# kdexd/virtex

Measured on NVIDIA H100. Metric: image-caption pairs/sec bicaptioning R50-L1-H1024, higher is better.
Workload: dtype bf16

## Files before the change

virtex_b200/csrc/gemm_tc.cu:

```cuda
#include <stdlib.h>
#include "ptx.cuh"
#include "vtx_common.cuh"
#include "../../include/virtex_b200.h"

#define KP_TAPS_W p.taps_w
#define KP_PAD p.pad
#define KP_NTAPS p.ntaps

namespace vtx {

constexpr int kBM = 128;
constexpr int kBK = 64;
constexpr int kMaxStages = 8;
constexpr int kABytes = kBM * kBK * 2;
constexpr int kSmemTotal = 232448;
constexpr int kCtrlBytes = 1024;
constexpr int kThreads = 384;
constexpr int kEpiThreads = 256;

struct FastDiv {
  uint32_t mul, shr;
};
__device__ __forceinline__ int fdiv(int x, const FastDiv& f) {
  return f.mul == 0u ? x : (int)(__umulhi((uint32_t)x, f.mul) >> f.shr);
// ... 18 lines not shown
  int bn;
  int a_mn, b_mn;
  int m_tiles, n_tiles, k_splits;
  int kb_total, kb_per_split;
  int mode;
  int cH, cW, cN, cpb;
  int lbw, lbh, lbn;
  int tiles_w, tiles_h;
  int out_f32, atomic, act;
  int stages, stage_bytes;
  int cbytes, nbuf;
  int res_tma;
  float alpha;
  void* D;
  long long ldd;
  const float* bias;
  int bias_pairs;
  const __nv_bfloat16* residual;
  long long ldr;
  const uint8_t* res_mask;
  float* stats;
  int taps_w, pad, ntaps;
  int cstride;
  FastDiv d_mn, d_nt, d_mt, d_tw, d_twh, d_cpb, d_taps;
  unsigned int* sched;
  unsigned int sched_base;
  int sched_chunk;
  int nt_major;
  const __nv_bfloat16* bnr_y;
  const float* bnr_bnp;
  const uint8_t* bnr_mask;
  long long bnr_ldy, bnr_sw, bnr_sh, bnr_sn;
  int vW, vH;
  int bnr_prefetch;
  int bnr;
  int trans_d;
  const float* col_scale;
  const float* col_shift;
};

__device__ __forceinline__ float gelu_erf(float x) { return 0.5f * x * (1.0f + erff(x * 0.70710678118654752f)); }

__device__ __forceinline__ void epi_bar(int id, int threads) {
  asm volatile("bar.sync %0, %1;" ::"r"(id), "r"(threads) : "memory");
}

__device__ __forceinline__ void decode_tile(const GemmKParams& p, int t, int& ks, int& mt, int& nt) {
  ks = fdiv(t, p.d_mn);
  const int rem = t - ks * (p.m_tiles * p.n_tiles);
  if (p.nt_major) {
    nt = fdiv(rem, p.d_mt);
    mt = rem - nt * p.m_tiles;
  } else {
    mt = fdiv(rem, p.d_nt);
    nt = rem - mt * p.n_tiles;
  }
}
__device__ __forceinline__ void tma_prefetch_l2_2d(const void* tmap, int c0, int c1) {
  asm volatile("cp.async.bulk.prefetch.tensor.2d.L2.global.tile [%0, {%1, %2}];" ::"l"(reinterpret_cast<uint64_t>(tmap)),
               "r"(c0), "r"(c1)
               : "memory");
}
__device__ __forceinline__ void tma_prefetch_l2_4d(const void* tmap, int c0, int c1, int c2, int c3) {
  asm volatile("cp.async.bulk.prefetch.tensor.4d.L2.global.tile [%0, {%1, %2, %3, %4}];" ::"l"(
                   reinterpret_cast<uint64_t>(tmap)),
               "r"(c0), "r"(c1), "r"(c2), "r"(c3)
               : "memory");
}
__device__ __forceinline__ uint4 ldg128_nc(const void* ptr) {
  uint4 v;
  asm volatile("ld.global.nc.L1::no_allocate.v4.b32 {%0, %1, %2, %3}, [%4];"
               : "=r"(v.x), "=r"(v.y), "=r"(v.z), "=r"(v.w)
               : "l"(ptr));
  return v;
}
constexpr int kSched = 8;

__device__ __forceinline__ uint32_t add_res_bf16x2(float lo, float hi, uint32_t res) {
  const __nv_bfloat162 a = __floats2bfloat162_rn(lo, hi);
  const __nv_bfloat162 r = *reinterpret_cast<const __nv_bfloat162*>(&res);
  const __nv_bfloat162 o = __hadd2(a, r);
  return *reinterpret_cast<const uint32_t*>(&o);
}
__device__ __forceinline__ void red_add_v2(float* addr, float a, float b) {
  asm volatile("red.global.add.v2.f32 [%0], {%1, %2};" ::"l"(addr), "f"(a), "f"(b) : "memory");
}
__device__ __forceinline__ uint32_t lds32(uint32_t saddr) {
  uint32_t v;
  asm volatile("ld.shared.b32 %0, [%1];" : "=r"(v) : "r"(saddr));
  return v;
}
__device__ __forceinline__ void sts32(uint32_t saddr, uint32_t v) {
  asm volatile("st.shared.b32 [%0], %1;" ::"r"(saddr), "r"(v) : "memory");
}
__device__ __forceinline__ uint32_t pack_bf16x2(float lo, float hi) {
  const __nv_bfloat162 h = __floats2bfloat162_rn(lo, hi);
  return *reinterpret_cast<const uint32_t*>(&h);
}

template <int BN, int TA, int TB>
__device__ __forceinline__ void wgmma_bn(float* d, uint64_t ad, uint64_t bd, uint32_t accumulate) {
// ... 11 lines not shown
  constexpr uint32_t b_step = TB ? 2048u : 32u;
  constexpr uint32_t a_lbo = TA ? 8192u : 16u;
  constexpr uint32_t b_lbo = TB ? 8192u : 16u;
  int prev = -1;
#pragma unroll
  for (int i = 0; i < NH * BN / 2; ++i) fence_operand(acc[i]);
  for (int kb = kb0; kb < kb1; ++kb) {
    mbar_wait(&full_bar[stage], phase);
    const uint32_t s0 = smem_u32(smem + stage * p.stage_bytes);
    const uint32_t sA = s0 + a_off;
    const uint32_t sB = s0 + (uint32_t)kABytes;
    wgmma_fence();
#pragma unroll
    for (int k = 0; k < kBK / 16; ++k) {
      const uint64_t bd = make_wgmma_desc(sB + k * b_step, b_lbo, 1024);
#pragma unroll
      for (int h = 0; h < NH; ++h)
        wgmma_bn<BN, TA, TB>(acc + h * (BN / 2), make_wgmma_desc(sA + h * 8192u + k * a_step, a_lbo, 1024), bd,
                             (kb > kb0 || k > 0) ? 1u : 0u);
    }
    wgmma_commit();
    wgmma_wait<1>();
    if (prev >= 0 && signal) mbar_arrive(&empty_bar[prev]);
    prev = stage;
    if (++stage == p.stages) { stage = 0; phase ^= 1; }
  }
  if (order_next != nullptr) mbar_arrive(order_next);
  wgmma_wait<0>();
  if (prev >= 0 && signal) mbar_arrive(&empty_bar[prev]);
#pragma unroll
  for (int i = 0; i < NH * BN / 2; ++i) fence_operand(acc[i]);
}

template <int BN, bool PP, bool SS>
__global__ void __launch_bounds__(kThreads, 1)
gemm_wgmma_kernel(const __grid_constant__ CUtensorMap tmA, const __grid_constant__ CUtensorMap tmB,
                  const __grid_constant__ CUtensorMap tmD, const __grid_constant__ CUtensorMap tmR,
                  const __grid_constant__ CUtensorMap tmY, const GemmKParams p) {
  static_assert(!PP || BN <= 128, "ping-pong tiles keep 2 x BN / 2 accumulators per thread");
  VTX_PDL_TRIGGER();
  extern __shared__ uint8_t smem_raw[];
  uint8_t* base = reinterpret_cast<uint8_t*>((reinterpret_cast<uintptr_t>(smem_raw) + 1023) & ~uintptr_t(1023));
  uint64_t* bars = reinterpret_cast<uint64_t*>(base);
  uint64_t* full_bar = bars;
  uint64_t* empty_bar = bars + kMaxStages;
  uint64_t* res_bar = bars + 2 * kMaxStages;
  uint64_t* sch_full = res_bar + 2;
  uint64_t* sch_empty = sch_full + kSched;
  uint64_t* order_bar = sch_empty + kSched;
  volatile unsigned long long* sch_tile = reinterpret_cast<volatile unsigned long long*>(order_bar + 2);
  uint8_t* smem = base + kCtrlBytes;
  uint8_t* cstage0 = smem + p.stages * p.stage_bytes;

  const int warp = __shfl_sync(0xffffffffu, (int)(threadIdx.x >> 5), 0);
  const int lane = threadIdx.x & 31;
  const int total_tiles = p.m_tiles * p.n_tiles * p.k_splits;
  const int nstages = p.stages;

  int t_first = blockIdx.x;
  if (warp == 0 && lane == 0) {
    if (p.sched != nullptr) t_first = (int)(atomicAdd(p.sched, 1u) - p.sched_base) * p.sched_chunk;
    tma_prefetch_desc(&tmA);
    tma_prefetch_desc(&tmB);
    if (p.cbytes) tma_prefetch_desc(&tmD);
    if (p.res_tma) tma_prefetch_desc(&tmR);
    if (p.bnr) tma_prefetch_desc(&tmY);
  }
  if (warp == 1 && lane == 0) {
    for (int i = 0; i < nstages; ++i) {
      mbar_init(&full_bar[i], 1);
      mbar_init(&empty_bar[i], PP ? 1 : 2);
    }
    for (int i = 0; i < 2; ++i) {
      mbar_init(&res_bar[i], 1);
      mbar_init(&order_bar[i], 128);
    }
    for (int i = 0; i < kSched; ++i) {
      mbar_init(&sch_full[i], 1);
      mbar_init(&sch_empty[i], PP ? 128 : kEpiThreads);
    }
    fence_mbar_init();
  }
  __syncthreads();
  VTX_PDL_WAIT();

  if (warp < 4) {
    setmaxnreg_dec<40>();
    if (warp == 0 && lane == 0) {
      const uint32_t b_bytes = (uint32_t)p.bn * kBK * 2;
      int stage = 0;
      uint32_t phase = 0;
      int t = t_first, sit = 0, kpos = 0;
      auto next_after = [&](int t_) -> int {
        if (p.sched == nullptr) return t_ + (int)gridDim.x;
        if ((t_ + 1) % p.sched_chunk != 0 && t_ + 1 < total_tiles) return t_ + 1;
        return (int)(atomicAdd(p.sched, 1u) - p.sched_base) * p.sched_chunk;
      };
      auto publish = [&](int t_) {
        const int slot = sit & (kSched - 1);
// ... 80 lines not shown
  const int wl = (ct >> 5) & 3;
  const bool signal = (ct & 127) == 0;
  constexpr int NH = PP ? 2 : 1;
  constexpr int epi_threads = PP ? 128 : kEpiThreads;
  const int bar_id = PP ? 1 + wg : 1;
  const int et = PP ? (ct & 127) : ct;
  const bool staged = p.cbytes != 0;
  const int st_lg = (p.bn == 64) ? 3 : (p.bn == 128) ? 4 : 5;
  const int st_rgs = min(epi_threads >> st_lg, 32), st_rpt = 128 / st_rgs;
  const int scg = et & ((1 << st_lg) - 1), srg = et >> st_lg;
  const bool st_on = (scg * 8 < p.bn) && (srg < st_rgs);
  float st_s[8], st_q[8];
#pragma unroll
  for (int i = 0; i < 8; ++i) st_s[i] = st_q[i] = 0.f;
  int st_nt = -1;
  auto flush_stats = [&](uint8_t* scratch) {
    float* scr = reinterpret_cast<float*>(scratch);
    if (st_on) {
#pragma unroll
      for (int i = 0; i < 8; i += 2) {
        *reinterpret_cast<float4*>(scr + (srg * p.bn + scg * 8 + i) * 2) =
            make_float4(st_s[i], st_q[i], st_s[i + 1], st_q[i + 1]);
        st_s[i] = st_q[i] = st_s[i + 1] = st_q[i + 1] = 0.f;
      }
    }
    epi_bar(bar_id, epi_threads);
    if (et < p.bn && st_nt * p.bn + et < p.N) {
      float a = 0.f, b = 0.f;
      for (int g = 0; g < st_rgs; ++g) {
        const float2 v = *reinterpret_cast<const float2*>(scr + (g * p.bn + et) * 2);
        a += v.x;
        b += v.y;
      }
      if (p.bnr) b *= __ldg(p.bnr_bnp + p.N + st_nt * p.bn + et);
      atomicAdd(p.stats + st_nt * p.bn + et, a);
      atomicAdd(p.stats + p.N + st_nt * p.bn + et, b);
    }
    epi_bar(bar_id, epi_threads);
  };
  auto issue_residual = [&](int t_, int bi_) {
    int ks_, mt_, nt_;
    decode_tile(p, t_, ks_, mt_, nt_);
    const int nb_ = nt_ * p.bn;
    uint8_t* buf_ = cstage0 + (size_t)bi_ * p.cbytes;
    const int slabs = (min(p.bn, p.N - nb_) + 63) >> 6;
    mbar_arrive_expect_tx(&res_bar[bi_], (uint32_t)slabs * 16384u);
    for (int sl = 0; sl < slabs; ++sl) {
      if (p.mode & 1) {
        const int tn_ = fdiv(mt_, p.d_twh);
        const int rwh_ = mt_ - tn_ * (p.tiles_w * p.tiles_h);
        const int th_ = fdiv(rwh_, p.d_tw), tw_ = rwh_ - th_ * p.tiles_w;
        tma_load_4d(buf_ + sl * 16384, &tmR, &res_bar[bi_], nb_ + sl * 64, tw_ << p.lbw, th_ << p.lbh, tn_ << p.lbn);
      } else {
        tma_load_2d(buf_ + sl * 16384, &tmR, &res_bar[bi_], nb_ + sl * 64, mt_ * kBM);
      }
    }
  };
  float acc[NH * BN / 2];
  for (int it = 0;; ++it) {
    const int sit = PP ? 2 * it + wg : it;
    const int slot = sit & (kSched - 1);
    mbar_wait(&sch_full[slot], (sit / kSched) & 1);
    const unsigned long long tk = sch_tile[slot];
    const int t = (int)(uint32_t)tk;
    const int kpos = (int)(tk >> 32);
    mbar_arrive(&sch_empty[slot]);
    if (t >= total_tiles) break;
    int ks, mt, nt;
    decode_tile(p, t, ks, mt, nt);
    const int n_base = nt * p.bn;
    int tw = 0, th = 0, tn = 0;
    if (p.mode & 1) {
      tn = fdiv(mt, p.d_twh);
      const int r_wh = mt - tn * (p.tiles_w * p.tiles_h);
      th = fdiv(r_wh, p.d_tw);
      tw = r_wh - th * p.tiles_w;
    }
    const int cbi = PP ? wg : p.nbuf > 1 ? (it & 1) : 0;
    uint8_t* cbuf = cstage0 + (size_t)cbi * p.cbytes;
    if (staged) {
      if (p.bnr && p.res_tma) epi_bar(bar_id, epi_threads);
      if (et == 0) {
        if (!PP && p.nbuf > 1) tma_store_wait_read<1>();
        else tma_store_wait_read<0>();
      }
      const bool new_block = p.stats != nullptr && st_nt != nt;
      if (new_block && st_nt >= 0 && p.res_tma) {
        epi_bar(bar_id, epi_threads);
        flush_stats(cbuf);
      }
      if (et == 0) {
        if (p.res_tma) issue_residual(t, cbi);
        if (p.bnr && p.bnr_prefetch) {
          const int slabs = (min(p.bn, p.N - n_base) + 63) >> 6;
          for (int sl = 0; sl < slabs; ++sl) {
            if (p.mode & 1) tma_prefetch_l2_4d(&tmY, n_base + sl * 64, tw << p.lbw, th << p.lbh, tn << p.lbn);
            else tma_prefetch_l2_2d(&tmY, n_base + sl * 64, mt * kBM);
          }
        }
      }
      epi_bar(bar_id, epi_threads);
      if (new_block) {
        if (st_nt >= 0 && !p.res_tma) flush_stats(cbuf);
        st_nt = nt;
      }
    }

    {
      const int kb0 = ks * p.kb_per_split;
      const int kb1 = min(p.kb_total, kb0 + p.kb_per_split);
      const int stage = kpos % p.stages;
      const uint32_t phase = (uint32_t)(kpos / p.stages) & 1u;
      const uint32_t a_off = PP ? 0u : (uint32_t)wg * 8192u;
      uint64_t* order_next = nullptr;
      if (PP) {
        if (wg == 1) mbar_wait(&order_bar[1], (uint32_t)it & 1u);
        else if (it > 0) mbar_wait(&order_bar[0], (uint32_t)(it - 1) & 1u);
        order_next = &order_bar[wg ^ 1];
      }
      if (!p.a_mn && !p.b_mn)
        mma_tile<BN, NH, 0, 0>(acc, smem, p, kb0, kb1, a_off, full_bar, empty_bar, stage, phase, signal, order_next);
      else if (!p.a_mn)
        mma_tile<BN, NH, 0, 1>(acc, smem, p, kb0, kb1, a_off, full_bar, empty_bar, stage, phase, signal, order_next);
      else if (!p.b_mn)
        mma_tile<BN, NH, 1, 0>(acc, smem, p, kb0, kb1, a_off, full_bar, empty_bar, stage, phase, signal, order_next);
      else
        mma_tile<BN, NH, 1, 1>(acc, smem, p, kb0, kb1, a_off, full_bar, empty_bar, stage, phase, signal, order_next);
    }
    if (p.res_tma) {
      const int uses = PP ? it : p.nbuf > 1 ? (it >> 1) : it;
      mbar_wait(&res_bar[cbi], uses & 1);
    }

    const int q = lane & 3;
    const bool plain = staged && !p.res_tma && p.bias == nullptr && p.residual == nullptr && p.act == 0 &&
                       p.alpha == 1.0f;
    const bool bias_only = staged && p.bias_pairs && p.residual == nullptr && p.act == 0 && p.alpha == 1.0f;
    const bool f32_only = !staged && p.bias == nullptr && p.residual == nullptr && p.act == 0;
    auto tile_row = [&](int r) -> long long {
      if (p.mode & 1) {
        const int dw = r & ((1 << p.lbw) - 1);
        const int dh = (r >> p.lbw) & ((1 << p.lbh) - 1);
        const int dn = r >> (p.lbw + p.lbh);
        const int w = (tw << p.lbw) + dw, h = (th << p.lbh) + dh, n = (tn << p.lbn) + dn;
        return (w < p.cW && h < p.cH && n < p.cN) ? ((long long)(n * p.cH + h) * p.cW + w) : -1;
      }
      const int r_ = mt * kBM + r;
      return r_ < p.M ? (long long)r_ : -1;
    };
    if constexpr (SS) {
      const uint32_t srow = smem_u32(cbuf) + ((PP ? 0 : wg) * 64 + wl * 16 + (lane >> 2)) * 128 + q * 4;
      const int sw = lane >> 2;
      const int col0 = n_base + 2 * q;
      const bool res = p.res_tma != 0, relu = p.act == 1;
#pragma unroll
      for (int j = 0; j < BN / 8; ++j) {
        const int col = col0 + 8 * j;
        const bool in = col < p.N;
        const float2 sc = in ? __ldg(reinterpret_cast<const float2*>(p.col_scale + col)) : make_float2(0.f, 0.f);
        const float2 sh = in ? __ldg(reinterpret_cast<const float2*>(p.col_shift + col)) : make_float2(0.f, 0.f);
        const uint32_t sa = srow + (j >> 3) * 16384 + (((j & 7) ^ sw) << 4);
#pragma unroll
// ... 141 lines not shown
          if (p.act == 1) {
            v0 = fmaxf(v0, 0.f);
            v1 = fmaxf(v1, 0.f);
          } else if (p.act == 2) {
            v0 = gelu_erf(v0);
            v1 = gelu_erf(v1);
          }
          if (staged) {
            sts32(sa, pack_bf16x2(v0, v1));
          } else if (grow >= 0) {
            float* D = reinterpret_cast<float*>(p.D);
            if (p.trans_d) {
              float* op = D + (long long)col * p.ldd + grow;
              atomicAdd(op, v0);
              if (two) atomicAdd(op + p.ldd, v1);
            } else {
              float* op = D + grow * p.ldd + col;
              if (p.atomic) {
                if (two) red_add_v2(op, v0, v1);
                else atomicAdd(op, v0);
              } else if (two) {
                *reinterpret_cast<float2*>(op) = make_float2(v0, v1);
              } else {
                op[0] = v0;
              }
            }
          }
        }
      }
    }

    const int bnr_r0 = srg * st_rpt;
    const int bnr_col = n_base + scg * 8;
    const bool bnr_on = p.bnr && st_on && bnr_col < p.N;
    auto bnr_load = [&](int rb, uint4* yv, uint32_t& mbits) {
      mbits = 0u;
#pragma unroll
      for (int r4 = 0; r4 < 4; ++r4) {
        const int r = bnr_r0 + rb + r4;
        uint32_t off, lin = 0;
        bool ok;
        if (p.mode & 1) {
          const int dw = r & ((1 << p.lbw) - 1);
          const int dh = (r >> p.lbw) & ((1 << p.lbh) - 1);
          const int dn = r >> (p.lbw + p.lbh);
          const int w = (tw << p.lbw) + dw, h = (th << p.lbh) + dh, n = (tn << p.lbn) + dn;
          ok = (w < p.vW) && (h < p.vH) && (n < p.cN);
          off = (uint32_t)n * (uint32_t)p.bnr_sn + (uint32_t)h * (uint32_t)p.bnr_sh + (uint32_t)w * (uint32_t)p.bnr_sw;
        } else {
          lin = (uint32_t)(mt * kBM + r);
          ok = lin < (uint32_t)p.M;
          off = lin * (uint32_t)p.bnr_ldy;
        }
        yv[r4] = ok ? ldg128_nc(p.bnr_y + off + bnr_col) : make_uint4(0u, 0u, 0u, 0u);
        const uint32_t mw = ok ? (p.bnr == 2 ? (uint32_t)__ldg(p.bnr_mask + ((lin * (uint32_t)p.N + bnr_col) >> 3)) : 0xffu) : 0u;
        mbits |= mw << (8 * r4);
      }
    };

    if (staged) {
      fence_proxy_async();
      epi_bar(bar_id, epi_threads);
      if (et == 0) {
        const int slabs = (min(p.bn, p.N - n_base) + 63) >> 6;
        for (int sl = 0; sl < slabs; ++sl) {
          if (p.mode & 1)
            tma_store_4d(&tmD, cbuf + sl * 16384, n_base + sl * 64, tw << p.lbw, th << p.lbh, tn << p.lbn);
          else
            tma_store_2d(&tmD, cbuf + sl * 16384, n_base + sl * 64, mt * kBM);
        }
        tma_store_commit();
      }
      if (bnr_on) {
        const uint32_t cp = smem_u32(cbuf) + (scg >> 3) * 16384 + bnr_r0 * 128;
        const int c8 = scg & 7;
        float mean[8], sc[8], sh[8];
        {
          const float4 m0 = __ldg(reinterpret_cast<const float4*>(p.bnr_bnp + bnr_col));
          const float4 m1 = __ldg(reinterpret_cast<const float4*>(p.bnr_bnp + bnr_col + 4));
          mean[0] = m0.x; mean[1] = m0.y; mean[2] = m0.z; mean[3] = m0.w;
          mean[4] = m1.x; mean[5] = m1.y; mean[6] = m1.z; mean[7] = m1.w;
          const float4 a0 = __ldg(reinterpret_cast<const float4*>(p.bnr_bnp + 2 * p.N + bnr_col));
          const float4 a1 = __ldg(reinterpret_cast<const float4*>(p.bnr_bnp + 2 * p.N + bnr_col + 4));
          const float4 b0 = __ldg(reinterpret_cast<const float4*>(p.bnr_bnp + 3 * p.N + bnr_col));
          const float4 b1 = __ldg(reinterpret_cast<const float4*>(p.bnr_bnp + 3 * p.N + bnr_col + 4));
          sc[0] = a0.x; sc[1] = a0.y; sc[2] = a0.z; sc[3] = a0.w; sc[4] = a1.x; sc[5] = a1.y; sc[6] = a1.z; sc[7] = a1.w;
          sh[0] = b0.x; sh[1] = b0.y; sh[2] = b0.z; sh[3] = b0.w; sh[4] = b1.x; sh[5] = b1.y; sh[6] = b1.z; sh[7] = b1.w;
        }
        for (int rb = 0; rb < st_rpt; rb += 4) {
          uint4 yv[4];
          uint32_t mbits;
          bnr_load(rb, yv, mbits);
#pragma unroll
          for (int r4 = 0; r4 < 4; ++r4) {
            const int r = rb + r4;
            const uint4 raw = lds128(cp + r * 128 + ((c8 ^ ((bnr_r0 + r) & 7)) << 4));
            float f[8], yy[8];
            unpack8(*reinterpret_cast<const bf16x8*>(&raw), f);
            unpack8(*reinterpret_cast<const bf16x8*>(&yv[r4]), yy);
#pragma unroll
            for (int i = 0; i < 8; ++i) {
              const bool on = p.bnr == 1 ? ((yy[i] * sc[i] + sh[i] > 0.f) && ((mbits >> (8 * r4)) & 0xffu) != 0u)
                                         : (((mbits >> (8 * r4 + i)) & 1u) != 0u);
              const float dz = on ? f[i] : 0.f;
              st_s[i] += dz;
              st_q[i] += dz * (yy[i] - mean[i]);
            }
          }
        }
      }
      if (!p.bnr && p.stats != nullptr && st_on) {
        const int r0 = srg * st_rpt;
        const uint32_t cp = smem_u32(cbuf) + (scg >> 3) * 16384 + r0 * 128;
        const int c8 = scg & 7;
        for (int rb = 0; rb < st_rpt; rb += 4) {
#pragma unroll
          for (int r4 = 0; r4 < 4; ++r4) {
            const int r = rb + r4;
            const uint4 raw = lds128(cp + r * 128 + ((c8 ^ ((r0 + r) & 7)) << 4));
            float f[8];
            unpack8(*reinterpret_cast<const bf16x8*>(&raw), f);
#pragma unroll
            for (int i = 0; i < 8; ++i) {
              st_s[i] += f[i];
              st_q[i] += f[i] * f[i];
            }
          }
        }
      }
    }
  }
  if (staged) {
    if (et == 0) tma_store_wait_read<0>();
    epi_bar(bar_id, epi_threads);
    if (p.stats != nullptr && st_nt >= 0) flush_stats(cstage0 + (PP ? (size_t)wg * p.cbytes : 0));
  }
}

typedef CUresult (*PFN_encodeTiled)(CUtensorMap*, CUtensorMapDataType, cuuint32_t, void*, const cuuint64_t*,
                                    const cuuint64_t*, const cuuint32_t*, const cuuint32_t*, CUtensorMapInterleave,
                                    CUtensorMapSwizzle, CUtensorMapL2promotion, CUtensorMapFloatOOBfill);

static PFN_encodeTiled get_encode() {
  static PFN_encodeTiled fn = nullptr;
// ... 53 lines not shown
    if (cudaMalloc(&ptr, sizeof(unsigned int) * kSchedSlots) != cudaSuccess) return nullptr;
    cudaMemset(ptr, 0, sizeof(unsigned int) * kSchedSlots);
    cudaDeviceSynchronize();
    memset(r.base, 0, sizeof(r.base));
    r.next = 0;
    r.ctr = ptr;
  }
  const unsigned int slot = r.next++ % kSchedSlots;
  *base_out = r.base[slot];
  r.base[slot] += fetches;
  return r.ctr + slot;
}

static int ilog2(int x) {
  int l = 0;
  while ((1 << l) < x) ++l;
  return l;
}

static void choose_box(int H, int W, int positions, int* bw, int* bh, int* bn) {
  int best_w = 1, best_h = 1;
  double best_eff = -1;
  for (int w = 1; w <= positions; w <<= 1)
    for (int h = 1; w * h <= positions; h <<= 1) {
      if (w > 2 * W || h > 2 * H) continue;
      const int tw = (W + w - 1) / w, th = (H + h - 1) / h;
      const double eff = (double)(W * H) / ((double)tw * w * th * h);
      const double score = eff * 1000.0 + w * 0.01 + h * 0.0001;
      if (score > best_eff) { best_eff = score; best_w = w; best_h = h; }
    }
  *bw = best_w; *bh = best_h; *bn = positions / (best_w * best_h);
}

template <bool SS>
static cudaError_t launch_gemm(const cudaLaunchConfig_t& cfg, bool pingpong, int bn, const CUtensorMap& tmA,
                               const CUtensorMap& tmB, const CUtensorMap& tmD, const CUtensorMap& tmR,
                               const CUtensorMap& tmY, const GemmKParams& p) {
  if (pingpong && bn == 64) return cudaLaunchKernelEx(&cfg, gemm_wgmma_kernel<64, true, SS>, tmA, tmB, tmD, tmR, tmY, p);
  if (pingpong) return cudaLaunchKernelEx(&cfg, gemm_wgmma_kernel<128, true, SS>, tmA, tmB, tmD, tmR, tmY, p);
  if (bn == 64) return cudaLaunchKernelEx(&cfg, gemm_wgmma_kernel<64, false, SS>, tmA, tmB, tmD, tmR, tmY, p);
  if (bn == 128) return cudaLaunchKernelEx(&cfg, gemm_wgmma_kernel<128, false, SS>, tmA, tmB, tmD, tmR, tmY, p);
  if (bn == 192) return cudaLaunchKernelEx(&cfg, gemm_wgmma_kernel<192, false, SS>, tmA, tmB, tmD, tmR, tmY, p);
  return cudaLaunchKernelEx(&cfg, gemm_wgmma_kernel<256, false, SS>, tmA, tmB, tmD, tmR, tmY, p);
}

}

using namespace vtx;

extern "C" int vtx_gemm_set_dynamic_schedule(int on) {
  g_sched_dynamic = on ? 1 : 0;
  return VTX_OK;
}

extern "C" int vtx_gemm(const VtxGemm* g, void* stream_) {
  cudaStream_t stream = reinterpret_cast<cudaStream_t>(stream_);
  if (!g || !g->A || !g->B || !g->D) return set_error(VTX_EINVAL, "vtx_gemm: null pointer");
  if (g->M <= 0 || g->N <= 0 || g->K <= 0) return set_error(VTX_EINVAL, "vtx_gemm: empty problem");
  if (g->atomic && !g->out_f32) return set_error(VTX_EINVAL, "vtx_gemm: atomic accumulate needs fp32 output");
  if (g->split_k > 1 && !g->atomic) return set_error(VTX_EINVAL, "vtx_gemm: split_k > 1 needs atomic = 1");
  if (g->stats && (g->out_f32 || g->bias || g->residual || g->act || (g->alpha != 0.f && g->alpha != 1.f)))
    return set_error(VTX_EINVAL, "vtx_gemm: stats needs a plain bf16 output (no bias/residual/activation/alpha)");
  if (g->ldd % (g->out_f32 ? 4 : 8) != 0) return set_error(VTX_EINVAL, "vtx_gemm: ldd must keep rows 16B aligned");
  if (g->conv_mode < 0 || g->conv_mode > 6 || g->conv_mode == 3)
    return set_error(VTX_EINVAL, "vtx_gemm: conv_mode must be 0, 1, 2, 4, 5 or 6");
  VtxGemm g4;
  const bool trans_d = g->conv_mode == 4;
  if (trans_d) {
    if (g->conv_c != 64 || g->N != 64 || g->M != 9 * 64 || !g->out_f32 || !g->atomic)
      return set_error(VTX_EINVAL, "vtx_gemm: conv_mode 4 needs C = Cout = 64, M = 576, fp32 atomic output");
    g4 = *g;
    g4.conv_mode = 2;
    g4.M = g->N;
    g4.N = g->M;
    g4.split_k = vtx_num_sms() / 3;
    g4.conv_stride = 1;
// ... 53 lines not shown
    return set_error(VTX_EINVAL, "vtx_gemm: bad tile_n %d", bn);
  bn = bn <= 64 ? 64 : bn <= 128 ? 128 : bn <= 192 ? 192 : 256;
  const bool pingpong = bn <= 128 && !g->out_f32;
  p.bn = bn;
  p.n_tiles = (g->N + bn - 1) / bn;
  p.trans_d = trans_d ? 1 : 0;
  p.out_f32 = g->out_f32; p.atomic = g->atomic; p.act = g->act;
  p.alpha = g->alpha == 0.f ? 1.0f : g->alpha;
  p.D = g->D; p.ldd = g->ldd;
  p.bias = g->bias;
  p.bias_pairs = (g->bias != nullptr && g->N % 2 == 0 && (reinterpret_cast<uintptr_t>(g->bias) & 7) == 0) ? 1 : 0;
  p.residual = reinterpret_cast<const __nv_bfloat16*>(g->residual);
  p.ldr = g->ldr;
  p.res_mask = reinterpret_cast<const uint8_t*>(g->residual_mask);
  if (p.res_mask != nullptr && (g->residual == nullptr || g->N % 32 != 0 || g->conv_mode != 0 || g->out_f32 ||
                                (reinterpret_cast<uintptr_t>(g->residual_mask) & 3) != 0))
    return set_error(VTX_EINVAL, "vtx_gemm: residual_mask needs a residual, a plain bf16 GEMM and N %% 32 == 0");
  p.stats = g->stats;
  const bool bnr = g->bnr_y != nullptr;
  if (bnr) {
    if (!g->bnr_bnp || !g->bnr_sums || g->stats || g->out_f32 || g->bias || g->act || (g->alpha != 0.f && g->alpha != 1.f) ||
        g->N % 8 != 0 || g->bnr_ldy % 8 != 0 || (reinterpret_cast<uintptr_t>(g->bnr_y) & 15) != 0 ||
        (reinterpret_cast<uintptr_t>(g->bnr_bnp) & 15) != 0 || (g->bnr_mask != nullptr && g->conv_mode != 0) ||
        g->conv_mode == 2 || g->conv_mode >= 4 || split_k > 1)
      return set_error(VTX_EINVAL, "vtx_gemm: bnr needs a plain bf16 output (no stats/bias/activation/alpha/split-K), "
                                   "N %% 8 == 0, 16-byte aligned y / bnp; the bit-mask form needs conv_mode 0");
    if ((long long)g->M * (g->bnr_ldy > g->N ? g->bnr_ldy : g->N) >= (1ll << 31))
      return set_error(VTX_EUNSUPPORTED, "vtx_gemm: bnr needs M * ld(y) < 2^31");
    p.stats = g->bnr_sums;
    p.bnr_y = reinterpret_cast<const __nv_bfloat16*>(g->bnr_y);
    p.bnr_bnp = g->bnr_bnp;
    p.bnr_mask = g->bnr_mask;
    p.bnr_ldy = g->bnr_ldy;
    const char* pf = getenv("VTX_BNR_PREFETCH");
    p.bnr_prefetch = (pf != nullptr && pf[0] == '0') ? 0 : 1;
    p.bnr = g->bnr_mask == nullptr ? 1 : 2;
  }
  const bool ss = g->col_scale != nullptr || g->col_shift != nullptr;
  if (ss) {
    if (!g->col_scale || !g->col_shift || g->out_f32 || (g->alpha != 0.f && g->alpha != 1.f) || g->bias || g->stats ||
        bnr || g->act < 0 || g->act > 1 || g->N % 2 != 0 || (reinterpret_cast<uintptr_t>(g->col_scale) & 7) != 0 ||
        (reinterpret_cast<uintptr_t>(g->col_shift) & 7) != 0 || g->residual_mask || g->conv_out_w > 0 ||
        (g->conv_mode != 0 && g->conv_mode != 1) ||
        (g->residual && (g->ldr % 8 != 0 || (reinterpret_cast<uintptr_t>(g->residual) & 15) != 0)))
      return set_error(VTX_EINVAL, "vtx_gemm: col_scale / col_shift need both vectors 8-byte aligned, a bf16 output, "
                                   "alpha 1, act 0 or 1, N %% 2 == 0, conv_mode 0 or 1 without an output view, no bias / "
                                   "stats / bnr / residual mask, and a 16-byte aligned residual with ldr %% 8 == 0");
    p.col_scale = g->col_scale;
    p.col_shift = g->col_shift;
  }

  CUtensorMap tmA, tmB;
  int rc;
  if (p.mode == 0) {
    p.m_tiles = (g->M + kBM - 1) / kBM;
    p.kb_total = (g->K + kBK - 1) / kBK;
    {
      uint64_t dims[2], str[1];
      uint32_t box[2];
      if (!p.a_mn) { dims[0] = g->K; dims[1] = g->M; box[0] = 64; box[1] = 128; }
      else { dims[0] = g->M; dims[1] = g->K; box[0] = 64; box[1] = 64; }
      str[0] = g->lda;
      if ((rc = make_tmap(&tmA, g->A, 2, dims, str, box)) != VTX_OK) return rc;
    }
    {
      uint64_t dims[2], str[1];
      uint32_t box[2];
      if (!p.b_mn) { dims[0] = g->K; dims[1] = g->N; box[0] = 64; box[1] = (uint32_t)bn; }
// ... 23 lines not shown
      p.kb_total = ntaps * p.cpb;
      uint32_t box[4] = {64, (uint32_t)(bw * cstride), (uint32_t)(bh * cstride), (uint32_t)bnn};
      const uint32_t es[4] = {1, (uint32_t)cstride, (uint32_t)cstride, 1};
      if ((rc = make_tmap(&tmA, g->A, 4, xdims, xstr, box, cstride > 1 ? es : nullptr)) != VTX_OK) return rc;
      uint64_t bd[2] = {(uint64_t)g->K, (uint64_t)g->N};
      uint64_t bs[1] = {(uint64_t)g->ldb};
      uint32_t bb[2] = {64, (uint32_t)bn};
      if ((rc = make_tmap(&tmB, g->B, 2, bd, bs, bb)) != VTX_OK) return rc;
    } else {
      if (g->N != ntaps * C) return set_error(VTX_EINVAL, "vtx_gemm: conv wgrad shape mismatch");
      const int Cout = g->M;
      if (Cout % 64 != 0) return set_error(VTX_EINVAL, "vtx_gemm: conv wgrad needs Cout %% 64 == 0");
      p.m_tiles = (Cout + kBM - 1) / kBM;
      p.kb_total = p.tiles_w * p.tiles_h * tiles_n;
      uint64_t ad[4] = {(uint64_t)Cout, (uint64_t)W, (uint64_t)H, (uint64_t)NI};
      uint64_t as[3] = {(uint64_t)Cout, (uint64_t)W * Cout, (uint64_t)H * W * Cout};
      uint32_t box[4] = {64, (uint32_t)bw, (uint32_t)bh, (uint32_t)bnn};
      if ((rc = make_tmap(&tmA, g->A, 4, ad, as, box)) != VTX_OK) return rc;
      uint32_t xbox[4] = {64, (uint32_t)(bw * cstride), (uint32_t)(bh * cstride), (uint32_t)bnn};
      const uint32_t es[4] = {1, (uint32_t)cstride, (uint32_t)cstride, 1};
      if ((rc = make_tmap(&tmB, g->B, 4, xdims, xstr, xbox, cstride > 1 ? es : nullptr)) != VTX_OK) return rc;
    }
  }
  p.k_splits = split_k;
  if (p.k_splits > p.kb_total) p.k_splits = p.kb_total;
  p.kb_per_split = (p.kb_total + p.k_splits - 1) / p.k_splits;
  p.k_splits = (p.kb_total + p.kb_per_split - 1) / p.kb_per_split;

  p.stage_bytes = kABytes + bn * kBK * 2;
  p.cbytes = p.out_f32 ? 0 : ((bn + 63) / 64) * 16384;
  {
    const int kb_tile = p.kb_per_split;
    const int budget = kSmemTotal - 1024  - kCtrlBytes;
    int st = 0;
    p.nbuf = 1;
    if (pingpong) {
      p.nbuf = 2;
    } else if (p.cbytes) {
      const int st2 = (budget - 2 * p.cbytes) / p.stage_bytes;
      if (st2 >= 4 || (st2 >= 2 && st2 >= kb_tile)) { p.nbuf = 2; st = st2; }
    }
    if (st == 0) st = (budget - p.nbuf * p.cbytes) / p.stage_bytes;
    if (st > kMaxStages) st = kMaxStages;
    if (st < 2) return set_error(VTX_EUNSUPPORTED, "vtx_gemm: not enough shared memory for a 2-stage pipeline");
    p.stages = st;
  }
  CUtensorMap tmD, tmR, tmY;
  memset(&tmY, 0, sizeof(tmY));
  memset(&tmD, 0, sizeof(tmD));
  memset(&tmR, 0, sizeof(tmR));
  p.res_tma = (p.cbytes && g->residual != nullptr && g->ldr % 8 == 0 &&
               (reinterpret_cast<uintptr_t>(g->residual) & 15) == 0 && p.alpha == 1.0f && g->bias == nullptr &&
               (g->act == 0 || ss)) ? 1 : 0;
  if (p.cbytes) {
    if (p.mode & 1) {
      uint64_t dd[4] = {(uint64_t)g->N, (uint64_t)p.cW, (uint64_t)p.cH, (uint64_t)g->conv_n};
      uint64_t ds[3] = {(uint64_t)g->ldd, (uint64_t)p.cW * g->ldd, (uint64_t)p.cH * p.cW * g->ldd};
      if (g->conv_out_w > 0) {
        if (g->conv_out_h <= 0 || g->ldd_w % 8 || g->ldd_h % 8 || g->ldd_n % 8 || (g->residual != nullptr && !p.res_tma))
          return set_error(VTX_EINVAL, "vtx_gemm: bad output view");
        dd[1] = (uint64_t)g->conv_out_w; dd[2] = (uint64_t)g->conv_out_h;
        ds[0] = (uint64_t)g->ldd_w; ds[1] = (uint64_t)g->ldd_h; ds[2] = (uint64_t)g->ldd_n;
      }
      uint32_t db[4] = {64, 1u << p.lbw, 1u << p.lbh, 1u << p.lbn};
      if ((rc = make_tmap(&tmD, g->D, 4, dd, ds, db)) != VTX_OK) return rc;
      p.vW = (int)dd[1]; p.vH = (int)dd[2];
      if (bnr) {
        uint64_t ys[3] = {(uint64_t)g->bnr_ldy, (uint64_t)p.cW * g->bnr_ldy, (uint64_t)p.cH * p.cW * g->bnr_ldy};
        if (g->conv_out_w > 0) { ys[0] = ds[0]; ys[1] = ds[1]; ys[2] = ds[2]; }
        p.bnr_sw = (long long)ys[0]; p.bnr_sh = (long long)ys[1]; p.bnr_sn = (long long)ys[2];
        if ((rc = make_tmap(&tmY, g->bnr_y, 4, dd, ys, db)) != VTX_OK) return rc;
      }
      if (p.res_tma) {
        uint64_t rs[3] = {(uint64_t)g->ldr, (uint64_t)p.cW * g->ldr, (uint64_t)p.cH * p.cW * g->ldr};
        if (g->conv_out_w > 0) { rs[0] = ds[0]; rs[1] = ds[1]; rs[2] = ds[2]; }
        if ((rc = make_tmap(&tmR, g->residual, 4, dd, rs, db)) != VTX_OK) return rc;
      }
    } else {
      uint64_t dd[2] = {(uint64_t)g->N, (uint64_t)g->M};
      uint64_t ds[1] = {(uint64_t)g->ldd};
      uint32_t db[2] = {64, 128};
      if ((rc = make_tmap(&tmD, g->D, 2, dd, ds, db)) != VTX_OK) return rc;
      if (bnr) {
        uint64_t ys[1] = {(uint64_t)g->bnr_ldy};
        if ((rc = make_tmap(&tmY, g->bnr_y, 2, dd, ys, db)) != VTX_OK) return rc;
      }
      if (p.res_tma) {
        uint64_t rs[1] = {(uint64_t)g->ldr};
        if ((rc = make_tmap(&tmR, g->residual, 2, dd, rs, db)) != VTX_OK) return rc;
      }
    }
  }
  {
    static bool attr_set[64] = {false};
    int dev = 0;
    cudaGetDevice(&dev);
    if (dev < 0 || dev >= 64 || !attr_set[dev]) {
      cudaError_t e = cudaSuccess;
      const void* kernels[12] = {
          (const void*)gemm_wgmma_kernel<64, false, false>,  (const void*)gemm_wgmma_kernel<128, false, false>,
          (const void*)gemm_wgmma_kernel<192, false, false>, (const void*)gemm_wgmma_kernel<256, false, false>,
          (const void*)gemm_wgmma_kernel<64, true, false>,   (const void*)gemm_wgmma_kernel<128, true, false>,
          (const void*)gemm_wgmma_kernel<64, false, true>,   (const void*)gemm_wgmma_kernel<128, false, true>,
          (const void*)gemm_wgmma_kernel<192, false, true>,  (const void*)gemm_wgmma_kernel<256, false, true>,
          (const void*)gemm_wgmma_kernel<64, true, true>,    (const void*)gemm_wgmma_kernel<128, true, true>};
      for (int i = 0; i < 12 && e == cudaSuccess; ++i)
        e = cudaFuncSetAttribute(kernels[i], cudaFuncAttributeMaxDynamicSharedMemorySize, kSmemTotal);
      if (e != cudaSuccess) return set_error(VTX_ECUDA, "cudaFuncSetAttribute: %s", cudaGetErrorString(e));
      if (dev >= 0 && dev < 64) attr_set[dev] = true;
    }
  }
  p.d_mn = make_fastdiv(p.m_tiles * p.n_tiles);
  p.d_nt = make_fastdiv(p.n_tiles);
  p.d_mt = make_fastdiv(p.m_tiles);
  p.nt_major = (p.stats != nullptr && p.n_tiles > 1) ? 1 : 0;
  const long total = (long)p.m_tiles * p.n_tiles * p.k_splits;
  const int sms = vtx_num_sms();
  const int grid = (int)(total < sms ? total : sms);
  p.sched_chunk = total >= 32L * grid ? 4 : total >= 12L * grid ? 2 : 1;
  const unsigned int fetches = (unsigned int)((total + p.sched_chunk - 1) / p.sched_chunk) + (unsigned int)grid;
  p.sched = sched_slot(fetches, &p.sched_base);
  p.d_tw = make_fastdiv(p.tiles_w);
  p.d_twh = make_fastdiv(p.tiles_w * p.tiles_h);
  p.d_cpb = make_fastdiv(p.cpb);
  p.d_taps = make_fastdiv(p.taps_w);
  {
    cudaLaunchConfig_t cfg;
    memset(&cfg, 0, sizeof(cfg));
    cfg.gridDim = dim3((unsigned)grid);
    cfg.blockDim = dim3(kThreads);
    cfg.dynamicSmemBytes = kSmemTotal;
    cfg.stream = stream;
    cudaLaunchAttribute attr[1];
    attr[0].id = cudaLaunchAttributeProgrammaticStreamSerialization;
    attr[0].val.programmaticStreamSerializationAllowed = 1;
    cfg.attrs = attr;
    cfg.numAttrs = 1;
    const cudaError_t le = ss ? launch_gemm<true>(cfg, pingpong, bn, tmA, tmB, tmD, tmR, tmY, p)
                              : launch_gemm<false>(cfg, pingpong, bn, tmA, tmB, tmD, tmR, tmY, p);
    if (le != cudaSuccess) return set_error(VTX_ECUDA, "gemm_wgmma_kernel PDL launch: %s", cudaGetErrorString(le));
  }
  cudaError_t e = cudaGetLastError();
  if (e != cudaSuccess) return set_error(VTX_ECUDA, "gemm_wgmma_kernel launch: %s", cudaGetErrorString(e));
  return VTX_OK;
}
```

Measured before the change: 5921.

## TMA-load BN-backward Y tiles into shared memory and specialize kernel on BNR

In the ping-pong GEMM epilogue used for BN-backward-ReLU fusion, the Y operand is now loaded by TMA into a dedicated shared-memory buffer alongside the residual. This replaces per-thread ldg loads that relied only on an L2 prefetch. A new BR template parameter compiles the BNR paths statically, and the dropout mask bytes are preloaded once per tile instead of inside the row loop. The extra shared-memory buffer can reduce the number of pipeline stages, so the host enables Y-TMA only when enough stages remain and otherwise falls back to the old layout.

Result: no change. 5961, median of 6 (+0.7%).

```diff
diff --git a/virtex_b200/csrc/gemm_tc.cu b/virtex_b200/csrc/gemm_tc.cu
--- a/virtex_b200/csrc/gemm_tc.cu
+++ b/virtex_b200/csrc/gemm_tc.cu
@@ -74,7 +74,7 @@
   const uint8_t* bnr_mask;
   long long bnr_ldy, bnr_sw, bnr_sh, bnr_sn;
   int vW, vH;
-  int bnr_prefetch;
+  int y_tma;
   int bnr;
   int trans_d;
   const float* col_scale;
@@ -98,17 +98,6 @@
     nt = rem - mt * p.n_tiles;
   }
 }
-__device__ __forceinline__ void tma_prefetch_l2_2d(const void* tmap, int c0, int c1) {
-  asm volatile("cp.async.bulk.prefetch.tensor.2d.L2.global.tile [%0, {%1, %2}];" ::"l"(reinterpret_cast<uint64_t>(tmap)),
-               "r"(c0), "r"(c1)
-               : "memory");
-}
-__device__ __forceinline__ void tma_prefetch_l2_4d(const void* tmap, int c0, int c1, int c2, int c3) {
-  asm volatile("cp.async.bulk.prefetch.tensor.4d.L2.global.tile [%0, {%1, %2, %3, %4}];" ::"l"(
-                   reinterpret_cast<uint64_t>(tmap)),
-               "r"(c0), "r"(c1), "r"(c2), "r"(c3)
-               : "memory");
-}
 __device__ __forceinline__ uint4 ldg128_nc(const void* ptr) {
   uint4 v;
   asm volatile("ld.global.nc.L1::no_allocate.v4.b32 {%0, %1, %2, %3}, [%4];"
@@ -186,12 +175,14 @@
   for (int i = 0; i < NH * BN / 2; ++i) fence_operand(acc[i]);
 }
 
-template <int BN, bool PP, bool SS>
+template <int BN, bool PP, bool SS, bool BR>
 __global__ void __launch_bounds__(kThreads, 1)
 gemm_wgmma_kernel(const __grid_constant__ CUtensorMap tmA, const __grid_constant__ CUtensorMap tmB,
                   const __grid_constant__ CUtensorMap tmD, const __grid_constant__ CUtensorMap tmR,
                   const __grid_constant__ CUtensorMap tmY, const GemmKParams p) {
   static_assert(!PP || BN <= 128, "ping-pong tiles keep 2 x BN / 2 accumulators per thread");
+  static_assert(!(SS && BR), "the scale / shift epilogue has no BN-backward reduction");
+  constexpr bool YT = BR && PP;
   VTX_PDL_TRIGGER();
   extern __shared__ uint8_t smem_raw[];
   uint8_t* base = reinterpret_cast<uint8_t*>((reinterpret_cast<uintptr_t>(smem_raw) + 1023) & ~uintptr_t(1023));
@@ -205,6 +196,7 @@
   volatile unsigned long long* sch_tile = reinterpret_cast<volatile unsigned long long*>(order_bar + 2);
   uint8_t* smem = base + kCtrlBytes;
   uint8_t* cstage0 = smem + p.stages * p.stage_bytes;
+  uint8_t* ystage0 = cstage0 + (size_t)p.nbuf * p.cbytes;
 
   const int warp = __shfl_sync(0xffffffffu, (int)(threadIdx.x >> 5), 0);
   const int lane = threadIdx.x & 31;
@@ -218,7 +210,7 @@
     tma_prefetch_desc(&tmB);
     if (p.cbytes) tma_prefetch_desc(&tmD);
     if (p.res_tma) tma_prefetch_desc(&tmR);
-    if (p.bnr) tma_prefetch_desc(&tmY);
+    if (BR) tma_prefetch_desc(&tmY);
   }
   if (warp == 1 && lane == 0) {
     for (int i = 0; i < nstages; ++i) {
@@ -365,30 +357,35 @@
         a += v.x;
         b += v.y;
       }
-      if (p.bnr) b *= __ldg(p.bnr_bnp + p.N + st_nt * p.bn + et);
+      if (BR) b *= __ldg(p.bnr_bnp + p.N + st_nt * p.bn + et);
       atomicAdd(p.stats + st_nt * p.bn + et, a);
       atomicAdd(p.stats + p.N + st_nt * p.bn + et, b);
     }
     epi_bar(bar_id, epi_threads);
   };
-  auto issue_residual = [&](int t_, int bi_) {
+  auto issue_operands = [&](int t_, int bi_) {
     int ks_, mt_, nt_;
     decode_tile(p, t_, ks_, mt_, nt_);
     const int nb_ = nt_ * p.bn;
-    uint8_t* buf_ = cstage0 + (size_t)bi_ * p.cbytes;
     const int slabs = (min(p.bn, p.N - nb_) + 63) >> 6;
-    mbar_arrive_expect_tx(&res_bar[bi_], (uint32_t)slabs * 16384u);
-    for (int sl = 0; sl < slabs; ++sl) {
-      if (p.mode & 1) {
-        const int tn_ = fdiv(mt_, p.d_twh);
-        const int rwh_ = mt_ - tn_ * (p.tiles_w * p.tiles_h);
-        const int th_ = fdiv(rwh_, p.d_tw), tw_ = rwh_ - th_ * p.tiles_w;
-        tma_load_4d(buf_ + sl * 16384, &tmR, &res_bar[bi_], nb_ + sl * 64, tw_ << p.lbw, th_ << p.lbh, tn_ << p.lbn);
-      } else {
-        tma_load_2d(buf_ + sl * 16384, &tmR, &res_bar[bi_], nb_ + sl * 64, mt_ * kBM);
-      }
-    }
+    const uint32_t tensors = (p.res_tma ? 1u : 0u) + (YT && p.y_tma ? 1u : 0u);
+    mbar_arrive_expect_tx(&res_bar[bi_], tensors * (uint32_t)slabs * 16384u);
+    auto load = [&](const CUtensorMap* tm, uint8_t* buf_) {
+      for (int sl = 0; sl < slabs; ++sl) {
+        if (p.mode & 1) {
+          const int tn_ = fdiv(mt_, p.d_twh);
+          const int rwh_ = mt_ - tn_ * (p.tiles_w * p.tiles_h);
+          const int th_ = fdiv(rwh_, p.d_tw), tw_ = rwh_ - th_ * p.tiles_w;
+          tma_load_4d(buf_ + sl * 16384, tm, &res_bar[bi_], nb_ + sl * 64, tw_ << p.lbw, th_ << p.lbh, tn_ << p.lbn);
+        } else {
+          tma_load_2d(buf_ + sl * 16384, tm, &res_bar[bi_], nb_ + sl * 64, mt_ * kBM);
+        }
+      }
+    };
+    if (p.res_tma) load(&tmR, cstage0 + (size_t)bi_ * p.cbytes);
+    if (YT && p.y_tma) load(&tmY, ystage0 + (size_t)bi_ * p.cbytes);
   };
+  const bool epi_loads = p.res_tma || (YT && p.y_tma);
   float acc[NH * BN / 2];
   for (int it = 0;; ++it) {
     const int sit = PP ? 2 * it + wg : it;
@@ -412,7 +409,7 @@
     const int cbi = PP ? wg : p.nbuf > 1 ? (it & 1) : 0;
     uint8_t* cbuf = cstage0 + (size_t)cbi * p.cbytes;
     if (staged) {
-      if (p.bnr && p.res_tma) epi_bar(bar_id, epi_threads);
+      if (BR && epi_loads) epi_bar(bar_id, epi_threads);
       if (et == 0) {
         if (!PP && p.nbuf > 1) tma_store_wait_read<1>();
         else tma_store_wait_read<0>();
@@ -422,16 +419,7 @@
         epi_bar(bar_id, epi_threads);
         flush_stats(cbuf);
       }
-      if (et == 0) {
-        if (p.res_tma) issue_residual(t, cbi);
-        if (p.bnr && p.bnr_prefetch) {
-          const int slabs = (min(p.bn, p.N - n_base) + 63) >> 6;
-          for (int sl = 0; sl < slabs; ++sl) {
-            if (p.mode & 1) tma_prefetch_l2_4d(&tmY, n_base + sl * 64, tw << p.lbw, th << p.lbh, tn << p.lbn);
-            else tma_prefetch_l2_2d(&tmY, n_base + sl * 64, mt * kBM);
-          }
-        }
-      }
+      if (et == 0 && epi_loads) issue_operands(t, cbi);
       epi_bar(bar_id, epi_threads);
       if (new_block) {
         if (st_nt >= 0 && !p.res_tma) flush_stats(cbuf);
@@ -460,7 +448,7 @@
       else
         mma_tile<BN, NH, 1, 1>(acc, smem, p, kb0, kb1, a_off, full_bar, empty_bar, stage, phase, signal, order_next);
     }
-    if (p.res_tma) {
+    if (epi_loads) {
       const int uses = PP ? it : p.nbuf > 1 ? (it >> 1) : it;
       mbar_wait(&res_bar[cbi], uses & 1);
     }
@@ -668,13 +656,22 @@
 
     const int bnr_r0 = srg * st_rpt;
     const int bnr_col = n_base + scg * 8;
-    const bool bnr_on = p.bnr && st_on && bnr_col < p.N;
-    auto bnr_load = [&](int rb, uint4* yv, uint32_t& mbits) {
-      mbits = 0u;
+    const bool bnr_on = BR && st_on && bnr_col < p.N;
+    uint32_t bmask[4] = {0u, 0u, 0u, 0u};
+    if (BR && p.bnr == 2 && bnr_on) {
+#pragma unroll
+      for (int r = 0; r < 16; ++r) {
+        const uint32_t lin = (uint32_t)(mt * kBM + bnr_r0 + r);
+        if (r < st_rpt && lin < (uint32_t)p.M)
+          bmask[r >> 2] |= (uint32_t)__ldg(p.bnr_mask + ((lin * (uint32_t)p.N + bnr_col) >> 3)) << (8 * (r & 3));
+      }
+    }
+    auto bnr_rows = [&](int rb, uint4* yv) -> uint32_t {
+      uint32_t mbits = 0u;
 #pragma unroll
       for (int r4 = 0; r4 < 4; ++r4) {
         const int r = bnr_r0 + rb + r4;
-        uint32_t off, lin = 0;
+        uint32_t off;
         bool ok;
         if (p.mode & 1) {
           const int dw = r & ((1 << p.lbw) - 1);
@@ -684,14 +681,14 @@
           ok = (w < p.vW) && (h < p.vH) && (n < p.cN);
           off = (uint32_t)n * (uint32_t)p.bnr_sn + (uint32_t)h * (uint32_t)p.bnr_sh + (uint32_t)w * (uint32_t)p.bnr_sw;
         } else {
-          lin = (uint32_t)(mt * kBM + r);
+          const uint32_t lin = (uint32_t)(mt * kBM + r);
           ok = lin < (uint32_t)p.M;
           off = lin * (uint32_t)p.bnr_ldy;
         }
-        yv[r4] = ok ? ldg128_nc(p.bnr_y + off + bnr_col) : make_uint4(0u, 0u, 0u, 0u);
-        const uint32_t mw = ok ? (p.bnr == 2 ? (uint32_t)__ldg(p.bnr_mask + ((lin * (uint32_t)p.N + bnr_col) >> 3)) : 0xffu) : 0u;
-        mbits |= mw << (8 * r4);
-      }
+        if (!(YT && p.y_tma)) yv[r4] = ok ? ldg128_nc(p.bnr_y + off + bnr_col) : make_uint4(0u, 0u, 0u, 0u);
+        mbits |= (ok ? 0xffu : 0u) << (8 * r4);
+      }
+      return mbits;
     };
 
     if (staged) {
@@ -709,6 +706,7 @@
       }
       if (bnr_on) {
         const uint32_t cp = smem_u32(cbuf) + (scg >> 3) * 16384 + bnr_r0 * 128;
+        const uint32_t yp = cp + (uint32_t)(p.nbuf * p.cbytes);
         const int c8 = scg & 7;
         float mean[8], sc[8], sh[8];
         {
@@ -725,15 +723,22 @@
         }
         for (int rb = 0; rb < st_rpt; rb += 4) {
           uint4 yv[4];
-          uint32_t mbits;
-          bnr_load(rb, yv, mbits);
+          uint32_t mbits = bnr_rows(rb, yv);
+          if (p.bnr == 2) {
+            mbits = bmask[0];
+            bmask[0] = bmask[1];
+            bmask[1] = bmask[2];
+            bmask[2] = bmask[3];
+          }
 #pragma unroll
           for (int r4 = 0; r4 < 4; ++r4) {
             const int r = rb + r4;
-            const uint4 raw = lds128(cp + r * 128 + ((c8 ^ ((bnr_r0 + r) & 7)) << 4));
+            const uint32_t so = r * 128 + ((c8 ^ ((bnr_r0 + r) & 7)) << 4);
+            const uint4 raw = lds128(cp + so);
+            const uint4 yraw = (YT && p.y_tma) ? lds128(yp + so) : yv[r4];
             float f[8], yy[8];
             unpack8(*reinterpret_cast<const bf16x8*>(&raw), f);
-            unpack8(*reinterpret_cast<const bf16x8*>(&yv[r4]), yy);
+            unpack8(*reinterpret_cast<const bf16x8*>(&yraw), yy);
 #pragma unroll
             for (int i = 0; i < 8; ++i) {
               const bool on = p.bnr == 1 ? ((yy[i] * sc[i] + sh[i] > 0.f) && ((mbits >> (8 * r4)) & 0xffu) != 0u)
@@ -745,7 +750,7 @@
           }
         }
       }
-      if (!p.bnr && p.stats != nullptr && st_on) {
+      if (!BR && p.stats != nullptr && st_on) {
         const int r0 = srg * st_rpt;
         const uint32_t cp = smem_u32(cbuf) + (scg >> 3) * 16384 + r0 * 128;
         const int c8 = scg & 7;
@@ -865,16 +870,17 @@
   *bw = best_w; *bh = best_h; *bn = positions / (best_w * best_h);
 }
 
-template <bool SS>
+template <bool SS, bool BR>
 static cudaError_t launch_gemm(const cudaLaunchConfig_t& cfg, bool pingpong, int bn, const CUtensorMap& tmA,
                                const CUtensorMap& tmB, const CUtensorMap& tmD, const CUtensorMap& tmR,
                                const CUtensorMap& tmY, const GemmKParams& p) {
-  if (pingpong && bn == 64) return cudaLaunchKernelEx(&cfg, gemm_wgmma_kernel<64, true, SS>, tmA, tmB, tmD, tmR, tmY, p);
-  if (pingpong) return cudaLaunchKernelEx(&cfg, gemm_wgmma_kernel<128, true, SS>, tmA, tmB, tmD, tmR, tmY, p);
-  if (bn == 64) return cudaLaunchKernelEx(&cfg, gemm_wgmma_kernel<64, false, SS>, tmA, tmB, tmD, tmR, tmY, p);
-  if (bn == 128) return cudaLaunchKernelEx(&cfg, gemm_wgmma_kernel<128, false, SS>, tmA, tmB, tmD, tmR, tmY, p);
-  if (bn == 192) return cudaLaunchKernelEx(&cfg, gemm_wgmma_kernel<192, false, SS>, tmA, tmB, tmD, tmR, tmY, p);
-  return cudaLaunchKernelEx(&cfg, gemm_wgmma_kernel<256, false, SS>, tmA, tmB, tmD, tmR, tmY, p);
+  if (pingpong && bn == 64)
+    return cudaLaunchKernelEx(&cfg, gemm_wgmma_kernel<64, true, SS, BR>, tmA, tmB, tmD, tmR, tmY, p);
+  if (pingpong) return cudaLaunchKernelEx(&cfg, gemm_wgmma_kernel<128, true, SS, BR>, tmA, tmB, tmD, tmR, tmY, p);
+  if (bn == 64) return cudaLaunchKernelEx(&cfg, gemm_wgmma_kernel<64, false, SS, BR>, tmA, tmB, tmD, tmR, tmY, p);
+  if (bn == 128) return cudaLaunchKernelEx(&cfg, gemm_wgmma_kernel<128, false, SS, BR>, tmA, tmB, tmD, tmR, tmY, p);
+  if (bn == 192) return cudaLaunchKernelEx(&cfg, gemm_wgmma_kernel<192, false, SS, BR>, tmA, tmB, tmD, tmR, tmY, p);
+  return cudaLaunchKernelEx(&cfg, gemm_wgmma_kernel<256, false, SS, BR>, tmA, tmB, tmD, tmR, tmY, p);
 }
 
 }
@@ -994,8 +1000,6 @@
     p.bnr_bnp = g->bnr_bnp;
     p.bnr_mask = g->bnr_mask;
     p.bnr_ldy = g->bnr_ldy;
-    const char* pf = getenv("VTX_BNR_PREFETCH");
-    p.bnr_prefetch = (pf != nullptr && pf[0] == '0') ? 0 : 1;
     p.bnr = g->bnr_mask == nullptr ? 1 : 2;
   }
   const bool ss = g->col_scale != nullptr || g->col_shift != nullptr;
@@ -1085,15 +1089,21 @@
   {
     const int kb_tile = p.kb_per_split;
     const int budget = kSmemTotal - 1024  - kCtrlBytes;
-    int st = 0;
-    p.nbuf = 1;
-    if (pingpong) {
-      p.nbuf = 2;
-    } else if (p.cbytes) {
-      const int st2 = (budget - 2 * p.cbytes) / p.stage_bytes;
-      if (st2 >= 4 || (st2 >= 2 && st2 >= kb_tile)) { p.nbuf = 2; st = st2; }
-    }
-    if (st == 0) st = (budget - p.nbuf * p.cbytes) / p.stage_bytes;
+    auto carve = [&](int buf_bytes) {
+      int st = 0;
+      p.nbuf = 1;
+      if (pingpong) {
+        p.nbuf = 2;
+      } else if (p.cbytes) {
+        const int st2 = (budget - 2 * buf_bytes) / p.stage_bytes;
+        if (st2 >= 4 || (st2 >= 2 && st2 >= kb_tile)) { p.nbuf = 2; st = st2; }
+      }
+      if (st == 0) st = (budget - p.nbuf * buf_bytes) / p.stage_bytes;
+      return st;
+    };
+    int st = carve(bnr ? 2 * p.cbytes : p.cbytes);
+    p.y_tma = bnr && pingpong && st >= 2 && (st >= 4 || kb_tile <= 8) ? 1 : 0;
+    if (bnr && !p.y_tma) st = carve(p.cbytes);
     if (st > kMaxStages) st = kMaxStages;
     if (st < 2) return set_error(VTX_EUNSUPPORTED, "vtx_gemm: not enough shared memory for a 2-stage pipeline");
     p.stages = st;
@@ -1150,14 +1160,17 @@
     cudaGetDevice(&dev);
     if (dev < 0 || dev >= 64 || !attr_set[dev]) {
       cudaError_t e = cudaSuccess;
-      const void* kernels[12] = {
-          (const void*)gemm_wgmma_kernel<64, false, false>,  (const void*)gemm_wgmma_kernel<128, false, false>,
-          (const void*)gemm_wgmma_kernel<192, false, false>, (const void*)gemm_wgmma_kernel<256, false, false>,
-          (const void*)gemm_wgmma_kernel<64, true, false>,   (const void*)gemm_wgmma_kernel<128, true, false>,
-          (const void*)gemm_wgmma_kernel<64, false, true>,   (const void*)gemm_wgmma_kernel<128, false, true>,
-          (const void*)gemm_wgmma_kernel<192, false, true>,  (const void*)gemm_wgmma_kernel<256, false, true>,
-          (const void*)gemm_wgmma_kernel<64, true, true>,    (const void*)gemm_wgmma_kernel<128, true, true>};
-      for (int i = 0; i < 12 && e == cudaSuccess; ++i)
+      const void* kernels[18] = {
+          (const void*)gemm_wgmma_kernel<64, false, false, false>,  (const void*)gemm_wgmma_kernel<128, false, false, false>,
+          (const void*)gemm_wgmma_kernel<192, false, false, false>, (const void*)gemm_wgmma_kernel<256, false, false, false>,
+          (const void*)gemm_wgmma_kernel<64, true, false, false>,   (const void*)gemm_wgmma_kernel<128, true, false, false>,
+          (const void*)gemm_wgmma_kernel<64, false, true, false>,   (const void*)gemm_wgmma_kernel<128, false, true, false>,
+          (const void*)gemm_wgmma_kernel<192, false, true, false>,  (const void*)gemm_wgmma_kernel<256, false, true, false>,
+          (const void*)gemm_wgmma_kernel<64, true, true, false>,    (const void*)gemm_wgmma_kernel<128, true, true, false>,
+          (const void*)gemm_wgmma_kernel<64, false, false, true>,   (const void*)gemm_wgmma_kernel<128, false, false, true>,
+          (const void*)gemm_wgmma_kernel<192, false, false, true>,  (const void*)gemm_wgmma_kernel<256, false, false, true>,
+          (const void*)gemm_wgmma_kernel<64, true, false, true>,    (const void*)gemm_wgmma_kernel<128, true, false, true>};
+      for (int i = 0; i < 18 && e == cudaSuccess; ++i)
         e = cudaFuncSetAttribute(kernels[i], cudaFuncAttributeMaxDynamicSharedMemorySize, kSmemTotal);
       if (e != cudaSuccess) return set_error(VTX_ECUDA, "cudaFuncSetAttribute: %s", cudaGetErrorString(e));
       if (dev >= 0 && dev < 64) attr_set[dev] = true;
@@ -1189,8 +1202,9 @@
     attr[0].val.programmaticStreamSerializationAllowed = 1;
     cfg.attrs = attr;
     cfg.numAttrs = 1;
-    const cudaError_t le = ss ? launch_gemm<true>(cfg, pingpong, bn, tmA, tmB, tmD, tmR, tmY, p)
-                              : launch_gemm<false>(cfg, pingpong, bn, tmA, tmB, tmD, tmR, tmY, p);
+    const cudaError_t le = ss    ? launch_gemm<true, false>(cfg, pingpong, bn, tmA, tmB, tmD, tmR, tmY, p)
+                           : bnr ? launch_gemm<false, true>(cfg, pingpong, bn, tmA, tmB, tmD, tmR, tmY, p)
+                                 : launch_gemm<false, false>(cfg, pingpong, bn, tmA, tmB, tmD, tmR, tmY, p);
     if (le != cudaSuccess) return set_error(VTX_ECUDA, "gemm_wgmma_kernel PDL launch: %s", cudaGetErrorString(le));
   }
   cudaError_t e = cudaGetLastError();
```
